# Tencent/PocketFlow

Measured on NVIDIA H100. Metric: images_per_sec_compression_aware_training_step, higher is better.
Workload: dtype f32

## Files before the change

pocketflow_b200/csrc/pf_conv_tma.cu:

```cuda
#include <cuda.h>

#include "pf_conv_tc.cuh"
#include "pf_tma.cuh"

namespace pfconv {
using namespace pftma;

constexpr int kTmaMaxStages = 8;
constexpr int kTmaThreads = (kMmaWarps + 1) * 32;
constexpr uint32_t kATileBytes = TM * 128;

struct TmaP {
  int M, Ng, BN, nk, n_tiles, total_tiles;
  int cblocks, R, S;
  int rows_hw, rows_w;
  int src_h, src_w;
  int base_w, base_h, str_w, str_h, flip;
  int na, nb;
  int accumulate, relu, ring, stage_budget;
  FastDiv d_hw, d_w, d_ntiles, d_cblocks, d_s;
  EpiAff aff;
  const pf_tc_act_hdr* a_hdr;
  const float* csum;
  int nseg;
  pf_tc_bn_out bn;
};

constexpr int kPingPongWarps = 4;
constexpr int kPingPongThreads = (kMmaWarps + 4) * 32;
constexpr int kProducerRegs = 40, kConsumerRegs = 232;

template <int AFF, int BN, int NA, int NB, bool BNO>
__device__ __forceinline__ void conv_tma_consumer(const TmaP& p, uint8_t* smem, uint32_t stage_bytes,
                                                  uint32_t n_stages, uint64_t* full_bar, uint64_t* empty_bar,
                                                  uint64_t* ml_bar, uint64_t* epi_bar, int* tab_n0, float* out,
                                                  const float* bias, const float* residual) {
  const int tid = threadIdx.x, warp = tid >> 5, lane = tid & 31;
  const int wg = warp >> 2, q = warp & 3, wtid = tid & 127;
  const uint32_t b_bytes = (uint32_t)BN * 128u;
  float* acc_s = reinterpret_cast<float*>(smem + p.stage_budget);
  long long* rowoff_all = reinterpret_cast<long long*>(acc_s + TM * acc_pitch(BN));
  float* jrow_all = reinterpret_cast<float*>(rowoff_all + kMmaWarps * 32);
  float* aff_tab = jrow_all + kMmaWarps * 32;
  uint8_t* ring_all = reinterpret_cast<uint8_t*>(aff_tab + (AFF == 2 ? 2 * 256 : (BNO ? 4 * kMaxBN : 0)));
  long long* rowoff = rowoff_all + warp * 32;
  float* jrow = jrow_all + warp * 32;
  uint8_t* ring = p.ring ? ring_all + (size_t)warp * p.ring * kRingSlotBytes : nullptr;
  const float* extra = residual ? residual : (p.accumulate ? out : nullptr);
  uint32_t it = (uint32_t)wg * (uint32_t)p.nk;
  for (int tile = blockIdx.x + wg * gridDim.x, j = 0; tile < p.total_tiles; tile += 2 * gridDim.x, ++j) {
    const bool wait_turn = wg == 1 || j > 0;
    const uint32_t turn_ph = (uint32_t)(wg == 1 ? j : j - 1) & 1u;
    if (wait_turn) mbar_wait_bounded(&ml_bar[wg], turn_ph);
    float acc[2][BN / 2];
#pragma unroll
    for (int h = 0; h < 2; ++h)
#pragma unroll
      for (int i = 0; i < BN / 2; ++i) acc[h][i] = 0.f;
    uint32_t s = it % n_stages, ph = (it / n_stages) & 1u, prev = 0;
    for (int ks = 0; ks < p.nk; ++ks) {
      mbar_wait_bounded(&full_bar[s], ph);
      const uint32_t a0 = smem_u32(smem + (size_t)s * stage_bytes), a1 = a0 + kATileBytes;
      const uint32_t b0 = a0 + (uint32_t)NA * kATileBytes, b1 = b0 + b_bytes;
      wgmma_fence();
#pragma unroll
      for (int kk = 0; kk < BK / 16; ++kk) {
        const uint64_t db0 = make_smem_desc(b0 + kk * 32, 16, 1024), db1 = make_smem_desc(b1 + kk * 32, 16, 1024);
#pragma unroll
        for (int h = 0; h < 2; ++h) {
          const uint32_t ha = (uint32_t)h * 64 * 128 + kk * 32;
          wg_mma_kslice<BN, 0, NA, NB>(acc[h], make_smem_desc(a0 + ha, 16, 1024), make_smem_desc(a1 + ha, 16, 1024),
                                       db0, db1);
        }
      }
      wgmma_commit();
      wgmma_wait<1>(acc);
      if (ks > 0) {
        __syncwarp();
        if (lane == 0) mbar_arrive(&empty_bar[prev]);
      }
      prev = s;
      if (++s == n_stages) { s = 0; ph ^= 1u; }
    }
    __syncwarp();
    if (lane == 0) mbar_arrive(&ml_bar[wg ^ 1]);
    wgmma_wait<0>(acc);
    if (p.nk > 0) {
      __syncwarp();
      if (lane == 0) mbar_arrive(&empty_bar[prev]);
    }
    it += 2u * (uint32_t)p.nk;
    const int mt = (int)fdiv((uint32_t)tile, p.d_ntiles);
    const int n0 = (tile - mt * p.n_tiles) * BN;
    const int m = mt * TM + q * 32 + lane;
    const long long off = m < p.M ? (long long)m * p.Ng : -1;
    float my_j = 0.f;
    if (AFF == 2 && p.csum && m < p.M) {
      const int img = (int)fdiv((uint32_t)m, p.d_hw);
      const int rem = m - img * p.rows_hw;
      const int y = (int)fdiv((uint32_t)rem, p.d_w), x = rem - y * p.rows_w;
      const int ow0 = p.base_w + x * p.str_w, oh0 = p.base_h + y * p.str_h;
      const int total = p.R * p.S * p.nseg;
      const float* cbase = p.csum + (size_t)img * p.src_h * p.src_w * p.nseg;
      auto term = [&](int u) -> float {
        if (u >= total) return 0.f;
        const int t = u / p.nseg, g = u - t * p.nseg;
        const int r = (int)fdiv((uint32_t)t, p.d_s), s_ = t - r * p.S;
        const int ih = oh0 + r, iw = ow0 + s_;
        const bool ok = (unsigned)ih < (unsigned)p.src_h && (unsigned)iw < (unsigned)p.src_w;
        return ok ? __ldg(cbase + ((size_t)ih * p.src_w + iw) * p.nseg + g) : 0.f;
      };
      float a0 = 0.f, a1 = 0.f, a2 = 0.f, a3 = 0.f;
      for (int u = 0; u < total; u += 4) {
        const float v0 = term(u), v1 = term(u + 1), v2 = term(u + 2), v3 = term(u + 3);
        a0 += v0; a1 += v1; a2 += v2; a3 += v3;
      }
      my_j = (a0 + a1) + (a2 + a3);
    }
    if (wait_turn) mbar_wait_bounded(&epi_bar[wg], turn_ph);
    wgmma_store_acc<BN>(acc[0], acc_s, acc_pitch(BN), 0, wtid);
    wgmma_store_acc<BN>(acc[1], acc_s, acc_pitch(BN), 64, wtid);
    constexpr bool TAB = AFF == 2 || BNO;
    const int tab_was = TAB ? *reinterpret_cast<volatile int*>(tab_n0) : 0;
    if (AFF == 2 && tab_was != n0) {
      const float a_s = p.aff.a_scale ? __ldg(p.aff.a_scale) : 1.f;
      for (int c = wtid; c < BN; c += 128) {
        const bool cok = n0 + c < p.Ng;
        const int bi = p.aff.per_channel ? n0 + c : 0;
        const float al = cok ? __ldg(p.aff.w_alpha + bi) : 0.f, be = cok ? __ldg(p.aff.w_beta + bi) : 0.f;
        const float sx = al * p.aff.w_rk;
        aff_tab[c] = sx * a_s;
        aff_tab[256 + c] = fmaf(p.aff.w_centre, sx, be) * a_s;
      }
    }
    if (BNO && tab_was != n0) bn_table(p.bn, aff_tab, n0, BN, p.Ng, wtid, 128);
    named_bar_sync(2 + wg, 128);
    if (TAB && tab_was != n0 && wtid == 0) *reinterpret_cast<volatile int*>(tab_n0) = n0;
    epilogue_rows<AFF, BNO>(acc_s + (size_t)(32 * q) * acc_pitch(BN), 0, 32, off, rowoff, out, extra, bias, p.relu, n0,
                            BN, p.Ng, lane, ring, p.aff, my_j, jrow, TAB ? aff_tab : nullptr, p.ring, p.bn);
    __syncwarp();
    if (lane == 0) mbar_arrive(&epi_bar[wg ^ 1]);
  }
}

template <int AFF, int BN, bool BNO = false>
__global__ void __launch_bounds__(kPingPongThreads, 1)
conv_tma_kernel(const __grid_constant__ CUtensorMap tmA0, const __grid_constant__ CUtensorMap tmA1,
                const __grid_constant__ CUtensorMap tmB0, const __grid_constant__ CUtensorMap tmB1,
                float* __restrict__ out, const float* __restrict__ bias, const float* __restrict__ residual,
                const __grid_constant__ TmaP p) {
  extern __shared__ uint8_t smem_raw[];
  uint8_t* smem = (uint8_t*)(((uintptr_t)smem_raw + 1023) & ~(uintptr_t)1023);
  __shared__ uint64_t full_bar[kTmaMaxStages], empty_bar[kTmaMaxStages], ml_bar[2], epi_bar[2];
  __shared__ int tab_n0;
  const int tid = threadIdx.x, warp = tid >> 5, lane = tid & 31;
  int na = p.na;
  if (p.a_hdr) na = (__ldg(&p.a_hdr->nplanes) == 2) ? 2 : 1;
  const int nb = p.nb;
  const uint32_t b_bytes = (uint32_t)BN * 128u;
  const uint32_t stage_bytes = (uint32_t)na * kATileBytes + (uint32_t)nb * b_bytes;
  const uint32_t n_stages = min((uint32_t)kTmaMaxStages, (uint32_t)p.stage_budget / stage_bytes);

  if (tid == 0) {
    for (int s = 0; s < kTmaMaxStages; ++s) {
      mbar_init(&full_bar[s], 1);
      mbar_init(&empty_bar[s], kPingPongWarps);
    }
    for (int w = 0; w < 2; ++w) {
      mbar_init(&ml_bar[w], kPingPongWarps);
      mbar_init(&epi_bar[w], kPingPongWarps);
    }
    tab_n0 = -1;
    fence_barrier_init();
  }
  __syncthreads();

  if (warp >= kMmaWarps) {
    setmaxnreg_dec<kProducerRegs>();
    if (warp == kMmaWarps && lane == 0) {
      prefetch_map(&tmA0);
      prefetch_map(&tmB0);
      if (na == 2) prefetch_map(&tmA1);
      if (nb == 2) prefetch_map(&tmB1);
      uint32_t s = 0, ph = 0;
      for (int tile = blockIdx.x; tile < p.total_tiles; tile += gridDim.x) {
        const int mt = (int)fdiv((uint32_t)tile, p.d_ntiles);
        const int n0 = (tile - mt * p.n_tiles) * BN;
        const int m0 = mt * TM;
        const int img = (int)fdiv((uint32_t)m0, p.d_hw);
        const int rem = m0 - img * p.rows_hw;
        const int y = (int)fdiv((uint32_t)rem, p.d_w), x = rem - y * p.rows_w;
        const int cw = p.base_w + x * p.str_w, ch = p.base_h + y * p.str_h;
        for (int ks = 0; ks < p.nk; ++ks) {
          mbar_wait_bounded(&empty_bar[s], ph ^ 1u);
          const int tap = (int)fdiv((uint32_t)ks, p.d_cblocks);
          const int cb = ks - tap * p.cblocks;
          const int r = (int)fdiv((uint32_t)tap, p.d_s), q = tap - r * p.S;
          const uint32_t ow = (uint32_t)(p.flip ? p.S - 1 - q : q), oh = (uint32_t)(p.flip ? p.R - 1 - r : r);
          const uint32_t sa = smem_u32(smem + (size_t)s * stage_bytes);
          const uint32_t sb = sa + (uint32_t)na * kATileBytes;
          mbar_arrive_expect_tx(&full_bar[s], stage_bytes);
          load_im2col(sa, &tmA0, &full_bar[s], cb * BK, cw, ch, img, ow, oh);
          if (na == 2) load_im2col(sa + kATileBytes, &tmA1, &full_bar[s], cb * BK, cw, ch, img, ow, oh);
          load_2d(sb, &tmB0, &full_bar[s], ks * BK, n0);
          if (nb == 2) load_2d(sb + b_bytes, &tmB1, &full_bar[s], ks * BK, n0);
          if (++s == n_stages) { s = 0; ph ^= 1u; }
        }
      }
    }
  } else {
    setmaxnreg_inc<kConsumerRegs>();
#define PF_TMA_CONSUMER(NA_, NB_)                                                                                    \
  conv_tma_consumer<AFF, BN, NA_, NB_, BNO>(p, smem, stage_bytes, n_stages, full_bar, empty_bar, ml_bar, epi_bar,     \
                                            &tab_n0, out, bias, residual)
    if (na == 2) {
      if (nb == 2) PF_TMA_CONSUMER(2, 2);
      else PF_TMA_CONSUMER(2, 1);
    } else {
      if (nb == 2) PF_TMA_CONSUMER(1, 2);
      else PF_TMA_CONSUMER(1, 1);
    }
#undef PF_TMA_CONSUMER
  }
}

struct WgTmaP {
  TcGeom g;
  int Mtot, Npix, pps, splits, BN, n_tiles, tiles, total_units;
  int na, nb, stage_budget;
  FastDiv d_pq, d_q, d_c, d_s, d_tiles, d_ntiles;
  EpiAff aff;
  const pf_tc_act_hdr* x_hdr;
};
constexpr uint32_t kWgBlockBytes = BK * 128;

template <int AFF, int BN>
__global__ void __launch_bounds__(kTmaThreads, 1)
conv_tma_wgrad_kernel(const __grid_constant__ CUtensorMap tmX0, const __grid_constant__ CUtensorMap tmX1,
                      const __grid_constant__ CUtensorMap tmY0, const __grid_constant__ CUtensorMap tmY1,
                      float* __restrict__ partial, const __grid_constant__ WgTmaP p) {
  extern __shared__ uint8_t smem_raw[];
  uint8_t* smem = (uint8_t*)(((uintptr_t)smem_raw + 1023) & ~(uintptr_t)1023);
  __shared__ uint64_t full_bar[kTmaMaxStages], empty_bar[kTmaMaxStages];
  const int tid = threadIdx.x, warp = tid >> 5, lane = tid & 31;
  const TcGeom& g = p.g;
  const int nblkB = BN / 64;
  int na = p.na;
  if (p.x_hdr) na = (__ldg(&p.x_hdr->nplanes) == 2) ? 2 : 1;
  const int nb = p.nb;
  const uint32_t a_bytes = 2 * kWgBlockBytes, b_bytes = (uint32_t)nblkB * kWgBlockBytes;
  const uint32_t stage_bytes = (uint32_t)na * a_bytes + (uint32_t)nb * b_bytes;
  const uint32_t n_stages = min((uint32_t)kTmaMaxStages, (uint32_t)p.stage_budget / stage_bytes);
  float* acc_s = reinterpret_cast<float*>(smem + p.stage_budget);
  long long* rowoff_all = reinterpret_cast<long long*>(acc_s + TM * acc_pitch(BN));
  float* jrow_all = reinterpret_cast<float*>(rowoff_all + kMmaWarps * 32);
  if (tid == 0) {
    for (int s = 0; s < kTmaMaxStages; ++s) {
      mbar_init(&full_bar[s], 1);
      mbar_init(&empty_bar[s], kMmaWarps);
    }
    fence_barrier_init();
  }
  __syncthreads();
  struct Unit {
    int split, m0, n0, pbeg, nk;
  };
  auto decode = [&](int u) -> Unit {
    Unit r;
    r.split = (int)fdiv((uint32_t)u, p.d_tiles);
    const int t = u - r.split * p.tiles;
    const int mt = (int)fdiv((uint32_t)t, p.d_ntiles);
    r.m0 = mt * TM;
    r.n0 = (t - mt * p.n_tiles) * BN;
    r.pbeg = r.split * p.pps;
    const int pend = min(p.Npix, r.pbeg + p.pps);
    r.nk = (pend - r.pbeg + BK - 1) / BK;
    return r;
  };

  if (warp == kMmaWarps) {
    if (lane == 0) {
      prefetch_map(&tmX0);
      prefetch_map(&tmY0);
      if (na == 2) prefetch_map(&tmX1);
      if (nb == 2) prefetch_map(&tmY1);
      const int pq = g.P * g.Q;
      uint32_t s = 0, ph = 0;
      for (int u = blockIdx.x; u < p.total_units; u += gridDim.x) {
        const Unit un = decode(u);
        int c0[2], tr[2], tq[2], nvalid = 0;
#pragma unroll
        for (int b = 0; b < 2; ++b) {
          const int kf = un.m0 + 64 * b;
          const int tap = (int)fdiv((uint32_t)kf, p.d_c);
          c0[b] = kf - tap * g.C;
          tr[b] = (int)fdiv((uint32_t)tap, p.d_s);
          tq[b] = tap - tr[b] * g.S;
          if (kf < p.Mtot) nvalid = b + 1;
        }
        const uint32_t tx = (uint32_t)na * (uint32_t)nvalid * kWgBlockBytes + (uint32_t)nb * b_bytes;
        for (int ks = 0; ks < un.nk; ++ks) {
          mbar_wait_bounded(&empty_bar[s], ph ^ 1u);
          const int pix0 = un.pbeg + ks * BK;
          const int pn = (int)fdiv((uint32_t)pix0, p.d_pq);
          const int rem = pix0 - pn * pq;
          const int oh = (int)fdiv((uint32_t)rem, p.d_q), ow = rem - oh * g.Q;
          const int cw = ow * g.sw - g.pl, ch = oh * g.sh - g.pt;
          const uint32_t sa = smem_u32(smem + (size_t)s * stage_bytes);
          const uint32_t sb = sa + (uint32_t)na * a_bytes;
          mbar_arrive_expect_tx(&full_bar[s], tx);
          for (int b = 0; b < nvalid; ++b) {
            load_im2col(sa + b * kWgBlockBytes, &tmX0, &full_bar[s], c0[b], cw, ch, pn, (uint32_t)tq[b], (uint32_t)tr[b]);
            if (na == 2)
              load_im2col(sa + a_bytes + b * kWgBlockBytes, &tmX1, &full_bar[s], c0[b], cw, ch, pn, (uint32_t)tq[b],
                          (uint32_t)tr[b]);
          }
          for (int j = 0; j < nblkB; ++j) {
            load_2d(sb + j * kWgBlockBytes, &tmY0, &full_bar[s], un.n0 + 64 * j, pix0);
            if (nb == 2) load_2d(sb + b_bytes + j * kWgBlockBytes, &tmY1, &full_bar[s], un.n0 + 64 * j, pix0);
          }
          if (++s == n_stages) { s = 0; ph ^= 1u; }
        }
      }
    }
  } else {
    const int wg = warp >> 2, q = warp & 3;
    long long* rowoff = rowoff_all + warp * 32;
    float* jrow = jrow_all + warp * 32;
    auto consume = [&](auto na_c, auto nb_c) {
    constexpr int NA = decltype(na_c)::value, NB = decltype(nb_c)::value;
    uint32_t s = 0, ph = 0;
    for (int u = blockIdx.x; u < p.total_units; u += gridDim.x) {
      const Unit un = decode(u);
      float acc[BN / 2];
#pragma unroll
      for (int i = 0; i < BN / 2; ++i) acc[i] = 0.f;
      uint32_t prev = 0;
      for (int ks = 0; ks < un.nk; ++ks) {
        mbar_wait_bounded(&full_bar[s], ph);
        const uint32_t base = smem_u32(smem + (size_t)s * stage_bytes);
        const uint32_t a0 = base + (uint32_t)wg * kWgBlockBytes, a1 = a0 + a_bytes;
        const uint32_t b0 = base + (uint32_t)NA * a_bytes, b1 = b0 + b_bytes;
        wg_mma_stage<BN, 1, NA, NB>(acc, a0, a1, b0, b1, 2048, 2048, kWgBlockBytes, 1024, kWgBlockBytes, 1024);
        wgmma_wait<1>(acc);
        if (ks > 0) {
          __syncwarp();
          if (lane == 0) mbar_arrive(&empty_bar[prev]);
        }
        prev = s;
        if (++s == n_stages) { s = 0; ph ^= 1u; }
      }
      wgmma_wait<0>(acc);
      if (un.nk > 0) {
        __syncwarp();
        if (lane == 0) mbar_arrive(&empty_bar[prev]);
      }
      const int em = un.m0 + q * 32 + lane;
      const long long off = em < p.Mtot ? ((long long)un.split * p.Mtot + em) * g.K : -1;
      wg_tile_to_smem<BN>(acc, acc_s, tid);
      epilogue_tile_a<AFF>(acc_s, warp, off, rowoff, partial, nullptr, nullptr, 0, un.n0, BN, g.K, lane, nullptr, p.aff,
                           0.f, jrow, pf_tc_bn_out{});
    }
    };
    using one = std::integral_constant<int, 1>;
    using two = std::integral_constant<int, 2>;
    if (na == 2) {
      if (nb == 2) consume(two(), two());
      else consume(two(), one());
    } else {
      if (nb == 2) consume(one(), two());
      else consume(one(), one());
    }
  }
}

static int g_feed_override = -1;
void conv_tma_set_feed(int mode) { g_feed_override = mode < 0 ? -1 : (mode ? 1 : 0); }
static bool tma_enabled() {
  if (g_feed_override >= 0) return g_feed_override == 1;
  static int on = -1;
  if (on < 0) {
    const char* v = getenv("PF_TC_FEED");
    on = !(v && strcmp(v, "lsu") == 0);
  }
  return on == 1;
}

bool conv_tma_eligible(int pass, const TcGeom& g) {
  if (!tma_enabled()) return false;
  if (pass == 0) return g.C % 64 == 0 && g.K % 16 == 0 && g.sh <= 8 && g.sw <= 8 && g.R <= 16 && g.S <= 16;
  if (pass == 1) return g.K % 64 == 0 && g.C % 16 == 0 && g.sh == 1 && g.sw == 1 && g.R <= 16 && g.S <= 16;
  return g.C % 64 == 0 && g.K % 64 == 0 && g.sh <= 8 && g.sw <= 8;
}

static int pick_bn(int Ng) {
  int BN = Ng >= 128 ? 128 : (Ng >= 64 ? 64 : (Ng >= 32 ? 32 : 16));
  const int forced = env_int("PF_TC_BN", 0);
  if (forced >= 16 && forced <= kMaxBN && forced <= ((Ng + 15) / 16) * 16 && (forced & (forced - 1)) == 0) BN = forced;
  return BN;
}

#define PF_TMA_ENCODE(call, who)                                                               \
  do {                                                                                         \
    const int e__ = (call);                                                                    \
    if (e__ != 0) {                                                                            \
      pf_set_error("%s: tensor-map encoding failed (%d): %s", who, e__, #call);                \
      return PF_ERR_INVALID_ARG;                                                               \
    }                                                                                          \
  } while (0)

int conv_tma_launch(int pass, const TcGeom& g, const pf_tc_act& a, const pf_tc_wt& w, float* out, int accumulate,
                    const float* bias, int relu, const float* residual, cudaStream_t st, const char* who,
                    const pf_tc_bn_out* bn) {
  TmaP p;
  memset(&p, 0, sizeof(p));
  const int CC = pass == 0 ? g.C : g.K;
  const int Hs = pass == 0 ? g.H : g.P, Ws = pass == 0 ? g.W : g.Q;
  const int Ho = pass == 0 ? g.P : g.H, Wo = pass == 0 ? g.Q : g.W;
  const int64_t M64 = (int64_t)g.N * Ho * Wo;
  PF_REQUIRE(M64 < (1ll << 31), "%s: too many rows", who);
  p.M = (int)M64;
  p.Ng = pass == 0 ? g.K : g.C;
  const int Kdim = g.R * g.S * CC;
  p.nk = Kdim / BK;
  p.cblocks = CC / BK;
  p.R = g.R;
  p.S = g.S;
  p.rows_hw = Ho * Wo;
  p.rows_w = Wo;
  p.src_h = Hs;
  p.src_w = Ws;
  if (pass == 0) {
    p.base_w = -g.pl; p.base_h = -g.pt; p.str_w = g.sw; p.str_h = g.sh; p.flip = 0;
  } else {
    p.base_w = g.pl - (g.S - 1); p.base_h = g.pt - (g.R - 1); p.str_w = 1; p.str_h = 1; p.flip = 1;
  }
  p.accumulate = accumulate;
  p.relu = relu;
  const int m_tiles = (p.M + TM - 1) / TM;
  const int BN = pick_bn(p.Ng);
  p.BN = BN;
  p.n_tiles = (p.Ng + BN - 1) / BN;
  p.total_tiles = m_tiles * p.n_tiles;
  p.d_hw = make_fastdiv((uint32_t)p.rows_hw);
  p.d_w = make_fastdiv((uint32_t)p.rows_w);
  p.d_ntiles = make_fastdiv((uint32_t)p.n_tiles);
  p.d_cblocks = make_fastdiv((uint32_t)p.cblocks);
  p.d_s = make_fastdiv((uint32_t)g.S);
  p.na = a.plane1 ? 2 : 1;
  p.nb = w.plane1 ? 2 : 1;
  p.a_hdr = a.hdr;
  PF_REQUIRE(a.hdr == nullptr || a.plane1 != nullptr, "%s: an operand with a device header needs both planes", who);
  int aff = 0;
  if (w.alpha) {
    PF_REQUIRE(w.beta != nullptr && w.bits >= 1 && w.bits <= 8, "%s: weight levels need alpha, beta and 1..8 bits", who);
    PF_REQUIRE(a.csum != nullptr && a.nseg >= 1, "%s: weight levels need the operand's channel sums", who);
    aff = 2;
    p.aff.w_alpha = w.alpha;
    p.aff.w_beta = w.beta;
    p.aff.per_channel = w.per_channel;
    p.aff.w_rk = 1.f / (float)((1 << w.bits) - 1);
    p.aff.w_centre = (float)(1 << (w.bits - 1));
    p.aff.a_scale = a.hdr ? &a.hdr->scale : nullptr;
    p.csum = a.csum;
    p.nseg = a.nseg;
  } else if (a.hdr) {
    aff = 1;
    p.aff.a_scale = &a.hdr->scale;
  }
  PF_REQUIRE(bn == nullptr || (pass == 0 && aff == 0), "%s: the folded batch norm needs a split-bf16 forward", who);
  if (bn) p.bn = *bn;
  const int stage_max = p.na * (int)kATileBytes + p.nb * BN * 128;
  const bool has_extra = residual != nullptr || accumulate;
  const int aff_tab_bytes = aff == 2 ? 2 * 256 * 4 : (bn ? 4 * kMaxBN * 4 : 0);
  const int epi_bytes = epi_fixed_bytes(BN) + aff_tab_bytes;
  int budget = (kSmemLimit - epi_bytes) / 1024 * 1024;
  int ring_bytes = 0;
  p.ring = 0;
  if (has_extra && env_int("PF_TC_RING", 1) && BN >= 64) {
    const int need = std::min(3, p.nk + 1);
    for (int depth = kRingDepth; depth >= 2 && !p.ring; depth >>= 1) {
      const int rb = kMmaWarps * depth * kRingSlotBytes;
      if ((budget - rb) / stage_max >= need) {
        p.ring = depth;
        ring_bytes = rb;
      }
    }
    if (p.ring) budget = (kSmemLimit - epi_bytes - ring_bytes) / 1024 * 1024;
  }
  PF_REQUIRE(budget / stage_max >= 2 || p.nk <= 1, "%s: shared-memory plan failed (BN %d)", who, BN);
  p.stage_budget = budget;
  const size_t smem = (size_t)budget + epi_bytes + (p.ring ? ring_bytes : 0);
  const int grid = std::min(p.total_tiles, PF_NUM_SMS);
  record_plan(pf_tc_plan{0, 1, pass, 0, BN, aff, p.na, p.nb, 0, p.ring, 0, budget, p.total_tiles, grid, 0, 0});
  if (p.total_tiles == 0) return PF_OK;
  alignas(64) CUtensorMap tA0, tA1, tB0, tB1;
  PF_TMA_ENCODE(encode_im2col_bf16(&tA0, a.plane0, g.N, Hs, Ws, CC, p.base_w, p.base_h, Wo, Ho, p.str_w, p.str_h, BK, TM), who);
  if (a.plane1)
    PF_TMA_ENCODE(encode_im2col_bf16(&tA1, a.plane1, g.N, Hs, Ws, CC, p.base_w, p.base_h, Wo, Ho, p.str_w, p.str_h, BK, TM), who);
  else
    tA1 = tA0;
  const int Kpad = pad64(Kdim);
  PF_TMA_ENCODE(encode_2d_bf16(&tB0, w.plane0, (uint64_t)Kpad, (uint64_t)p.Ng, (uint64_t)Kpad, BK, (uint32_t)BN), who);
  if (w.plane1)
    PF_TMA_ENCODE(encode_2d_bf16(&tB1, w.plane1, (uint64_t)Kpad, (uint64_t)p.Ng, (uint64_t)Kpad, BK, (uint32_t)BN), who);
  else
    tB1 = tB0;
  cudaError_t err = cudaSuccess;
  with_bn(BN, [&](auto bn_c) {
    constexpr int B = decltype(bn_c)::value;
    auto kern = bn ? conv_tma_kernel<0, B, true>
                   : (aff == 2 ? conv_tma_kernel<2, B> : (aff == 1 ? conv_tma_kernel<1, B> : conv_tma_kernel<0, B>));
    err = cudaFuncSetAttribute(kern, cudaFuncAttributeMaxDynamicSharedMemorySize, (int)smem);
    if (err == cudaSuccess) kern<<<grid, kPingPongThreads, smem, st>>>(tA0, tA1, tB0, tB1, out, bias, residual, p);
  });
  PF_CUDA(err);
  PF_CHECK_LAUNCH(who);
  return PF_OK;
}

int conv_tma_wgrad_launch(const TcGeom& g, const pf_tc_act& x, const pf_tc_act& dy, int BN, int pps, int splits,
                          float* partial, cudaStream_t st, const char* who) {
  WgTmaP p;
  memset(&p, 0, sizeof(p));
  p.g = g;
  p.Mtot = g.R * g.S * g.C;
  p.Npix = g.N * g.P * g.Q;
  p.BN = BN;
  p.pps = pps;
  p.splits = splits;
  const int m_tiles = (p.Mtot + TM - 1) / TM;
  p.n_tiles = (g.K + BN - 1) / BN;
  p.tiles = m_tiles * p.n_tiles;
  p.total_units = p.tiles * p.splits;
  p.d_pq = make_fastdiv((uint32_t)(g.P * g.Q));
  p.d_q = make_fastdiv((uint32_t)g.Q);
  p.d_c = make_fastdiv((uint32_t)g.C);
  p.d_s = make_fastdiv((uint32_t)g.S);
  p.d_tiles = make_fastdiv((uint32_t)p.tiles);
  p.d_ntiles = make_fastdiv((uint32_t)p.n_tiles);
  p.na = x.plane1 ? 2 : 1;
  p.nb = dy.plane1 ? 2 : 1;
  p.x_hdr = x.hdr;
  PF_REQUIRE(x.hdr == nullptr || x.plane1 != nullptr, "%s: an operand with a device header needs both planes", who);
  PF_REQUIRE(dy.hdr == nullptr, "%s: the gradient operand is always split-bf16", who);
  int aff = 0;
  if (x.hdr) {
    aff = 1;
    p.aff.a_scale = &x.hdr->scale;
  }
  const int stage_max = p.na * 2 * (int)kWgBlockBytes + p.nb * (BN / 64) * (int)kWgBlockBytes;
  const int budget = (kSmemLimit - epi_fixed_bytes(BN)) / 1024 * 1024;
  PF_REQUIRE(budget / stage_max >= 2, "%s: shared-memory plan failed (BN %d)", who, BN);
  p.stage_budget = budget;
  const size_t smem = (size_t)budget + epi_fixed_bytes(BN);
  const int grid = std::min(p.total_units, PF_NUM_SMS);
  record_plan(pf_tc_plan{0, 1, 2, 0, BN, aff, p.na, p.nb, 0, 0, 0, budget, p.total_units, grid, splits, pps});
  if (p.total_units == 0) return PF_OK;
  alignas(64) CUtensorMap tX0, tX1, tY0, tY1;
  PF_TMA_ENCODE(encode_im2col_bf16(&tX0, x.plane0, g.N, g.H, g.W, g.C, -g.pl, -g.pt, g.Q, g.P, g.sw, g.sh, BK, BK), who);
  if (x.plane1)
    PF_TMA_ENCODE(encode_im2col_bf16(&tX1, x.plane1, g.N, g.H, g.W, g.C, -g.pl, -g.pt, g.Q, g.P, g.sw, g.sh, BK, BK), who);
  else
    tX1 = tX0;
  PF_TMA_ENCODE(encode_2d_bf16(&tY0, dy.plane0, (uint64_t)g.K, (uint64_t)p.Npix, (uint64_t)g.K, BK, BK), who);
  if (dy.plane1)
    PF_TMA_ENCODE(encode_2d_bf16(&tY1, dy.plane1, (uint64_t)g.K, (uint64_t)p.Npix, (uint64_t)g.K, BK, BK), who);
  else
    tY1 = tY0;
  auto kern = BN == 128 ? (aff == 1 ? conv_tma_wgrad_kernel<1, 128> : conv_tma_wgrad_kernel<0, 128>)
                        : (aff == 1 ? conv_tma_wgrad_kernel<1, 64> : conv_tma_wgrad_kernel<0, 64>);
  PF_CUDA(cudaFuncSetAttribute(kern, cudaFuncAttributeMaxDynamicSharedMemorySize, (int)smem));
  kern<<<grid, kTmaThreads, smem, st>>>(tX0, tX1, tY0, tY1, partial, p);
  PF_CHECK_LAUNCH(who);
  return PF_OK;
}

}
```

Baseline: 2660.

## Chunk BN=128 epilogue through a 32-column staging buffer to free pipeline stages

For BN=128 tiles with no affine, batch-norm or residual epilogue, the accumulators are now staged to shared memory 32 columns at a time rather than as a full 128-column tile. This shrinks the epilogue staging area, so the freed shared memory can hold an extra TMA pipeline stage when the plan would otherwise have fewer than three. The cost is extra named barriers and four epilogue passes per tile. It only activates when the stage count actually increases.

```diff
diff --git a/pocketflow_b200/csrc/pf_conv_tma.cu b/pocketflow_b200/csrc/pf_conv_tma.cu
--- a/pocketflow_b200/csrc/pf_conv_tma.cu
+++ b/pocketflow_b200/csrc/pf_conv_tma.cu
@@ -18,6 +18,7 @@
   int base_w, base_h, str_w, str_h, flip;
   int na, nb;
   int accumulate, relu, ring, stage_budget;
+  int chunked;
   FastDiv d_hw, d_w, d_ntiles, d_cblocks, d_s;
   EpiAff aff;
   const pf_tc_act_hdr* a_hdr;
@@ -29,6 +30,29 @@
 constexpr int kPingPongWarps = 4;
 constexpr int kPingPongThreads = (kMmaWarps + 4) * 32;
 constexpr int kProducerRegs = 40, kConsumerRegs = 232;
+
+__device__ __forceinline__ void conv_tma_epilogue_chunked(float (&acc)[2][64], const TmaP& p, float* acc_s,
+                                                          int n0, long long off, long long* rowoff, float* out,
+                                                          const float* bias, int wg, int q, int lane) {
+  constexpr int P = acc_pitch(32);
+  float* r0 = acc_s + (size_t)(16 * q + (lane >> 2)) * P + 2 * (lane & 3);
+#pragma unroll
+  for (int ch = 0; ch < 4; ++ch) {
+    if (ch > 0) named_bar_sync(2 + wg, 128);
+#pragma unroll
+    for (int h = 0; h < 2; ++h)
+#pragma unroll
+      for (int jj = 0; jj < 4; ++jj) {
+        const int j = 4 * ch + jj;
+        *reinterpret_cast<float2*>(r0 + (size_t)(64 * h) * P + 8 * jj) = make_float2(acc[h][4 * j], acc[h][4 * j + 1]);
+        *reinterpret_cast<float2*>(r0 + (size_t)(64 * h + 8) * P + 8 * jj) =
+            make_float2(acc[h][4 * j + 2], acc[h][4 * j + 3]);
+      }
+    named_bar_sync(2 + wg, 128);
+    epilogue_rows<0>(acc_s + (size_t)(32 * q) * P, 0, 32, off, rowoff, out, nullptr, bias, p.relu, n0 + 32 * ch, 32,
+                     p.Ng, lane, nullptr, p.aff, 0.f, nullptr, nullptr, 0, p.bn);
+  }
+}
 
 template <int AFF, int BN, int NA, int NB, bool BNO>
 __device__ __forceinline__ void conv_tma_consumer(const TmaP& p, uint8_t* smem, uint32_t stage_bytes,
@@ -39,7 +63,7 @@
   const int wg = warp >> 2, q = warp & 3, wtid = tid & 127;
   const uint32_t b_bytes = (uint32_t)BN * 128u;
   float* acc_s = reinterpret_cast<float*>(smem + p.stage_budget);
-  long long* rowoff_all = reinterpret_cast<long long*>(acc_s + TM * acc_pitch(BN));
+  long long* rowoff_all = reinterpret_cast<long long*>(acc_s + TM * acc_pitch(p.chunked ? 32 : BN));
   float* jrow_all = reinterpret_cast<float*>(rowoff_all + kMmaWarps * 32);
   float* aff_tab = jrow_all + kMmaWarps * 32;
   uint8_t* ring_all = reinterpret_cast<uint8_t*>(aff_tab + (AFF == 2 ? 2 * 256 : (BNO ? 4 * kMaxBN : 0)));
@@ -118,9 +142,17 @@
       my_j = (a0 + a1) + (a2 + a3);
     }
     if (wait_turn) mbar_wait_bounded(&epi_bar[wg], turn_ph);
+    constexpr bool TAB = AFF == 2 || BNO;
+    if constexpr (BN == 128 && AFF == 0 && !BNO) {
+      if (p.chunked) {
+        conv_tma_epilogue_chunked(acc, p, acc_s, n0, off, rowoff, out, bias, wg, q, lane);
+        __syncwarp();
+        if (lane == 0) mbar_arrive(&epi_bar[wg ^ 1]);
+        continue;
+      }
+    }
     wgmma_store_acc<BN>(acc[0], acc_s, acc_pitch(BN), 0, wtid);
     wgmma_store_acc<BN>(acc[1], acc_s, acc_pitch(BN), 64, wtid);
-    constexpr bool TAB = AFF == 2 || BNO;
     const int tab_was = TAB ? *reinterpret_cast<volatile int*>(tab_n0) : 0;
     if (AFF == 2 && tab_was != n0) {
       const float a_s = p.aff.a_scale ? __ldg(p.aff.a_scale) : 1.f;
@@ -488,9 +520,20 @@
     }
     if (p.ring) budget = (kSmemLimit - epi_bytes - ring_bytes) / 1024 * 1024;
   }
+  int used_epi = epi_bytes;
+  p.chunked = 0;
+  if (BN == 128 && aff == 0 && !bn && !has_extra && p.nk >= 3) {
+    const int chunk_epi = epi_fixed_bytes(32);
+    const int chunk_budget = (kSmemLimit - chunk_epi) / 1024 * 1024;
+    if (budget / stage_max < 3 && chunk_budget / stage_max > budget / stage_max) {
+      p.chunked = 1;
+      budget = chunk_budget;
+      used_epi = chunk_epi;
+    }
+  }
   PF_REQUIRE(budget / stage_max >= 2 || p.nk <= 1, "%s: shared-memory plan failed (BN %d)", who, BN);
   p.stage_budget = budget;
-  const size_t smem = (size_t)budget + epi_bytes + (p.ring ? ring_bytes : 0);
+  const size_t smem = (size_t)budget + used_epi + (p.ring ? ring_bytes : 0);
   const int grid = std::min(p.total_tiles, PF_NUM_SMS);
   record_plan(pf_tc_plan{0, 1, pass, 0, BN, aff, p.na, p.nb, 0, p.ring, 0, budget, p.total_tiles, grid, 0, 0});
   if (p.total_tiles == 0) return PF_OK;
```

Measured after the change: 2746 (median of 6 runs). 3.2% higher.
